# yunqing-me/RICK

Hardware: AMD Instinct MI355X
Metric: G+D train-step images/sec @256px (higher is better)
Workload: dtype f32 (fp16x3 split MFMA, fp32 accumulate); 1 GPU; FFHQ-256 StyleGAN2 G+D RICK iteration (D step, R1/16, G step, PLR/4, EMA, masks on), batch 4/GPU, 256px, channel_multiplier 2, random-init weights; global_batch=4, parallelism=dp1, hip_graphs=True

## Files before the change

include/rick_hip.h:

```cpp
#ifndef RICK_HIP_H
#define RICK_HIP_H

#include <stdint.h>

#ifdef __cplusplus
extern "C" {
#endif

#define RICK_EINVAL 22
#define RICK_MAX_TAPS 16

int rick_abi_version(void);

int rick_upfirdn2d_f32(const float *input, const float *kernel, float *out,
                       int64_t major, int in_h, int in_w, int minor, int kh, int kw,
                       int up_x, int up_y, int down_x, int down_y,
                       int pad_x0, int pad_x1, int pad_y0, int pad_y1, void *stream);

int rick_upfirdn2d_any(const void *input, const void *kernel, void *out, int dtype, int64_t major, int in_h, int in_w,
                       int kh, int kw, int up_x, int up_y, int down_x, int down_y, int pad_x0, int pad_x1, int pad_y0,
                       int pad_y1, void *stream);

int rick_bias_act_f32(const float *x, const float *bias, const float *ref, float *out,
                      int64_t n, int64_t step_b, int64_t size_b, int act, int grad,
// ... 146 lines not shown
int rick_conv_igemm_split_f32(const void *x_split, const float *x_hdr, const void *packed_w, float *out,
                              const float *oscale, const rick_conv_geom *g, const rick_conv_epilogue *epilogue,
                              void *workspace, void *stream);
int rick_convt2_split_f32(const void *x_split, const float *x_hdr, const void *packed_w, float *out, const float *oscale,
                          int N, int IH, int IW, int Ci, int Co, int OH, int OW, float alpha, float *amax ,
                          void *workspace, void *stream);
int rick_conv_wgrad_split_f32(const void *x, const float *x_hdr, const void *gy, const float *gy_hdr, float *gw,
                              int64_t s_co, int64_t s_ci, int64_t s_t, const rick_conv_geom *g, int accumulate,
                              void *workspace, void *stream);

int rick_thin_fwd_f32(const float *x, const float *W, int64_t w_bstride, const float *add,
                      float *t, int N, int64_t P, int C, int J, void *stream);
int rick_thin_bwdx_f32(const float *t, const float *W, int64_t w_bstride, float *x,
                       int N, int64_t P, int C, int J, void *stream);
int rick_torgb_fwd_f32(const float *x, const float *w, const float *s, float wscale, const float *bias,
                       const float *add, float *t, int N, int64_t P, int C, int J, void *stream);
int rick_torgb_bwdx_f32(const float *g, const float *w, const float *s, float wscale, float *gx, int N, int64_t P,
                        int C, int J, void *stream);
int rick_torgb_bwdx_acc_f32(const float *g, const float *w, const float *s, float wscale, float *gx, int N, int64_t P,
                            int C, int J, void *stream);
int rick_thin_wgrad_blocks(int64_t P);
int rick_thin_wgrad_f32(const float *t, const float *x, float *G, int N, int64_t P, int C, int J,
                        float *partials, void *stream);

int rick_chan_scale_f32(const float *x, const float *s, float *y, int N, int64_t P, int C, void *stream);
int rick_hw_dot_blocks(int64_t P);
int rick_hw_dot_f32(const float *a, const float *b, float *d, int N, int64_t P, int C,
                    float *partials, const float *divisor, void *stream);
int rick_hw_dot_scale_f32(const float *a, const float *b, float *d, const float *scale, float *scaled, int N,
                          int64_t P, int C, float *partials, void *stream);
int rick_hw_dot_act_f32(const float *g, const float *y, float *d, int N, int64_t P, int C, const float *bias,
                        const float *noise, const float *noise_w, int noise_nb, float slope, float gain,
                        float *partials, const float *divisor, void *stream);
int rick_add_scale_f32(const float *a, const float *b, float *y, int64_t n, float alpha, void *stream);

int rick_mbstd_fwd_f32(const float *x, float *out, float *stat, int B, int P, int C, int groups, void *stream);
int rick_mbstd_bwd_f32(const float *x, const float *gout, float *gx, int B, int P, int C, int groups, void *stream);

int rick_sq_accumulate_f32(float *acc, const float *g, int64_t n, void *stream);
int rick_filter_reduce_f32(const float *x, float *out, int64_t outer, int64_t outer_stride,
                           int64_t nfilters, int64_t filter_stride, int64_t inner,
                           float scale, void *stream);
int rick_wsq_f32(const float *w, float *wsq, int O, int I, int K, float scale, void *stream);
int rick_demod_f32(const float *s, const float *wsq, float *d, int B, int I, int O, float eps, void *stream);
int rick_demod_bwd_s_f32(const float *s, const float *wsq, const float *d, const float *gd, float *gs, int B, int I, int O,
                         void *stream);
int rick_demod_bwd_w_f32(const float *w, const float *s, const float *d, const float *gd, float *gw, int B, int I, int O,
                         int K, float scale, int accumulate, void *stream);
typedef struct {
    const float *w;
    const float *b;
    int64_t io_off;
    int64_t gw_off, gb_off;
    int C, lat_idx, blk_begin, reserved;
} rick_modbank_desc;
int rick_modbank_blocks(int C);
int rick_modbank_fwd_f32(const float *lat, int B, int n_latent, int K, const rick_modbank_desc *descs_device, int n,
                         int total_blocks, float scale, float *out, void *stream);
int rick_modbank_bwd_f32(const float *lat, const float *gs, int B, int n_latent, int K, const rick_modbank_desc *descs_device,
                         int n, int total_blocks, float scale, float *grad, int accumulate, void *stream);
typedef struct rick_demod_desc {
    const float *w;
    float *wsq;
    float *gw;
    int64_t s_off, d_off;
    int O, I, K;
// ... 134 lines not shown
```

rick_amd/_lib.py:

```python
import ctypes
import os

import torch

_HERE = os.path.dirname(os.path.abspath(__file__))
LIB_PATH = os.path.join(_HERE, 'lib', 'librick_hip.so')
if os.environ.get('RICK_HIP_LIB'):
    import warnings
    LIB_PATH = os.environ['RICK_HIP_LIB']
    warnings.warn(f'rick_amd: RICK_HIP_LIB overrides the product library with {LIB_PATH}', RuntimeWarning)
MAX_TAPS = 16

c_fp = ctypes.c_void_p
c_i64 = ctypes.c_int64
c_int = ctypes.c_int
c_f = ctypes.c_float


class ConvGeom(ctypes.Structure):
    _fields_ = [('N', c_int), ('IH', c_int), ('IW', c_int), ('Ci', c_int),
                ('OH', c_int), ('OW', c_int), ('Co', c_int),
                ('GH', c_int), ('GW', c_int),
                ('is_', c_int), ('os', c_int), ('oy0', c_int), ('ox0', c_int),
                ('ntaps', c_int), ('nslices', c_int),
# ... 71 lines not shown
    'rick_bound_tail_f32': (c_int, [c_fp, c_fp, c_f, c_fp, c_fp, c_fp, c_int, c_f, c_fp, c_int, c_fp]),
    'rick_bias_act_bwd_split2_f32': (c_int, [c_fp, c_fp, c_fp, c_fp, c_fp, c_fp, c_f, c_fp, c_fp, c_fp, c_fp, c_fp, c_fp, c_fp, c_i64,
                                             c_int, c_i64, c_i64, c_i64, c_f, c_f, c_fp, c_int, c_fp]),
    'rick_conv_packed_bytes': (c_i64, [c_int, c_int, c_int]),
    'rick_conv_pack_weight': (c_int, [c_fp, c_i64, c_i64, c_i64, c_int, c_int, c_int, c_f, c_int, c_fp, c_fp]),
    'rick_conv_pack_blocks': (c_int, [c_int, c_int]),
    'rick_conv_pack_weights_multi': (c_int, [c_fp, c_int, c_int, c_int, c_fp]),
    'rick_conv_igemm_workspace_bytes': (c_i64, [ctypes.POINTER(ConvGeom)]),
    'rick_conv_igemm_f32': (c_int, [c_fp, c_fp, c_fp, c_fp, c_fp, ctypes.POINTER(ConvGeom), c_fp, c_fp]),
    'rick_conv_igemm_act_f32': (c_int, [c_fp, c_fp, c_fp, c_fp, c_fp, ctypes.POINTER(ConvGeom),
                                        ctypes.POINTER(ConvEpilogue), c_fp, c_fp]),
    'rick_conv_igemm_multi_workspace_bytes': (c_i64, [ctypes.POINTER(ConvGeom), c_int]),
    'rick_conv_igemm_multi_f32': (c_int, [c_fp, c_fp, c_fp, c_fp, c_fp, ctypes.POINTER(ConvGeom), c_int, c_fp, c_fp]),
    'rick_convt2_workspace_bytes': (c_i64, [c_int] * 7),
    'rick_convt2_plan': (c_int, [c_int] * 7 + [ctypes.POINTER(c_int)]),
    'rick_convt2_posmap': (c_int, [c_int] * 7 + [ctypes.POINTER(ctypes.c_ubyte), ctypes.POINTER(c_int)]),
    'rick_convt2_f32': (c_int, [c_fp, c_fp, c_fp, c_fp, c_fp] + [c_int] * 8 + [c_f, c_fp, c_fp]),
    'rick_conv_wgrad_workspace_bytes': (c_i64, [ctypes.POINTER(ConvGeom)]),
    'rick_conv_wgrad_f32': (c_int, [c_fp, c_fp, c_fp, c_i64, c_i64, c_i64, c_fp, c_fp,
                                    ctypes.POINTER(ConvGeom), c_int, c_fp, c_fp]),
    'rick_thin_fwd_f32': (c_int, [c_fp, c_fp, c_i64, c_fp, c_fp, c_int, c_i64, c_int, c_int, c_fp]),
    'rick_thin_bwdx_f32': (c_int, [c_fp, c_fp, c_i64, c_fp, c_int, c_i64, c_int, c_int, c_fp]),
    'rick_torgb_fwd_f32': (c_int, [c_fp, c_fp, c_fp, c_f, c_fp, c_fp, c_fp, c_int, c_i64, c_int, c_int, c_fp]),
    'rick_torgb_bwdx_f32': (c_int, [c_fp, c_fp, c_fp, c_f, c_fp, c_int, c_i64, c_int, c_int, c_fp]),
    'rick_torgb_bwdx_acc_f32': (c_int, [c_fp, c_fp, c_fp, c_f, c_fp, c_int, c_i64, c_int, c_int, c_fp]),
    'rick_thin_wgrad_blocks': (c_int, [c_i64]),
    'rick_thin_wgrad_f32': (c_int, [c_fp, c_fp, c_fp, c_int, c_i64, c_int, c_int, c_fp, c_fp]),
    'rick_chan_scale_f32': (c_int, [c_fp, c_fp, c_fp, c_int, c_i64, c_int, c_fp]),
    'rick_hw_dot_blocks': (c_int, [c_i64]),
    'rick_hw_dot_f32': (c_int, [c_fp, c_fp, c_fp, c_int, c_i64, c_int, c_fp, c_fp, c_fp]),
    'rick_hw_dot_scale_f32': (c_int, [c_fp, c_fp, c_fp, c_fp, c_fp, c_int, c_i64, c_int, c_fp, c_fp]),
    'rick_hw_dot_act_f32': (c_int, [c_fp, c_fp, c_fp, c_int, c_i64, c_int, c_fp, c_fp, c_fp, c_int, c_f, c_f, c_fp, c_fp,
                                    c_fp]),
    'rick_add_scale_f32': (c_int, [c_fp, c_fp, c_fp, c_i64, c_f, c_fp]),
    'rick_mbstd_fwd_f32': (c_int, [c_fp, c_fp, c_fp, c_int, c_int, c_int, c_int, c_fp]),
    'rick_mbstd_bwd_f32': (c_int, [c_fp, c_fp, c_fp, c_int, c_int, c_int, c_int, c_fp]),
    'rick_sq_accumulate_f32': (c_int, [c_fp, c_fp, c_i64, c_fp]),
    'rick_filter_reduce_f32': (c_int, [c_fp, c_fp, c_i64, c_i64, c_i64, c_i64, c_i64, c_f, c_fp]),
    'rick_masked_adam_f32': (c_int, [c_fp, c_fp, c_fp, c_fp, c_fp, c_i64, c_f, c_f, c_f, c_f, c_f, c_f, c_fp]),
    'rick_wsq_f32': (c_int, [c_fp, c_fp, c_int, c_int, c_int, c_f, c_fp]),
    'rick_demod_f32': (c_int, [c_fp, c_fp, c_fp, c_int, c_int, c_int, c_f, c_fp]),
    'rick_demod_bwd_s_f32': (c_int, [c_fp, c_fp, c_fp, c_fp, c_fp, c_int, c_int, c_int, c_fp]),
    'rick_demod_bwd_w_f32': (c_int, [c_fp, c_fp, c_fp, c_fp, c_fp, c_int, c_int, c_int, c_int, c_f, c_int, c_fp]),
    'rick_colsum_multi_f32': (c_int, [ctypes.POINTER(ColsumItem), c_int, c_fp]),
    'rick_demod_blocks_wsq': (c_int, [c_int, c_int]),
    'rick_demod_blocks': (c_int, [c_int]),
    'rick_demod_blocks_bwd_s': (c_int, [c_int]),
    'rick_wsq_multi_f32': (c_int, [c_fp, c_int, c_int, c_fp]),
    'rick_demod_multi_f32': (c_int, [c_fp, c_fp, c_fp, c_int, c_int, c_int, c_int, c_f, c_fp]),
    'rick_demod_bwd_w_multi_f32': (c_int, [c_fp, c_fp, c_fp, c_fp, c_int, c_int, c_int, c_fp]),
    'rick_demod_bwd_s_multi_f32': (c_int, [c_fp, c_fp, c_fp, c_fp, c_fp, c_int, c_int, c_int, c_int, c_fp]),
    'rick_modbank_blocks': (c_int, [c_int]),
    'rick_modbank_fwd_f32': (c_int, [c_fp, c_int, c_int, c_int, c_fp, c_int, c_int, c_f, c_fp, c_fp]),
    'rick_modbank_bwd_f32': (c_int, [c_fp, c_fp, c_int, c_int, c_int, c_fp, c_int, c_int, c_f, c_fp, c_int, c_fp]),
    'rick_equal_linear_f32': (c_int, [c_fp, c_fp, c_fp, c_fp, c_int, c_int, c_int, c_f, c_f, c_int, c_f, c_f, c_int, c_fp]),
    'rick_linear_fwd_workspace_floats': (c_i64, [c_int, c_int, c_int]),
    'rick_linear_fwd_f32': (c_int, [c_fp, c_fp, c_fp, c_fp, c_int, c_int, c_int, c_f, c_f, c_fp, c_fp]),
    'rick_linear_dgrad_workspace_floats': (c_i64, [c_int, c_int, c_int]),
    'rick_linear_dgrad_f32': (c_int, [c_fp, c_fp, c_fp, c_int, c_int, c_int, c_f, c_fp, c_fp]),
    'rick_linear_wgrad_f32': (c_int, [c_fp, c_fp, c_fp, c_fp, c_int, c_int, c_int, c_f, c_f, c_int, c_fp]),
    'rick_adam_prepare_f32': (c_int, [c_fp, c_int, c_int, c_f, c_f, c_fp, c_fp]),
    'rick_masked_adam_dev_f32': (c_int, [c_fp, c_fp, c_fp, c_fp, c_fp, c_i64, c_f, c_f, c_f, c_f, c_fp, c_fp]),
    'rick_ema_f32': (c_int, [c_fp, c_fp, c_i64, c_f, c_fp]),
    'rick_image_batch_f32': (c_int, [c_fp, c_fp, c_fp, c_fp, c_int, c_int, c_int, c_int, c_fp]),
    'rick_png_unfilter': (c_int, [c_fp, c_int, c_int, c_int]),
    'rick_augment_workspace_floats': (c_i64, [c_int, c_int, c_int]),
# ... 106 lines not shown
```

rick_amd/csrc/elementwise.hip:

```cpp
#include "conv_common.h"

struct BiasActParams {
    int64_t n, step_b, size_b, n_div, hw_div, noise_nb, noise_hw;
    int act, grad;
    float alpha, scale;
};

__device__ __forceinline__ float act_apply(float v, float r, int mode, float alpha) {
    switch (mode) {
        case 30: return v > 0.f ? v : v * alpha;
        case 31: return r > 0.f ? v : v * alpha;
        case 12:
        case 32: return 0.f;
        default: return v;
    }
}

template <bool VEC4>
__global__ __launch_bounds__(256) void bias_act_kernel(const float *__restrict__ x, const float *__restrict__ b,
                                                       const float *__restrict__ ref, float *__restrict__ out,
                                                       const float *__restrict__ noise, const float *__restrict__ nw,
                                                       BiasActParams p) {
    const int mode = p.act * 10 + p.grad;
    const float nwv = noise ? nw[0] : 0.f;
// ... 676 lines not shown
    else
        hipLaunchKernelGGL((hw_dot_kernel<false, false>), dim3(nb, N), dim3(256), 1024 * sizeof(float), st, a, b, partials, P, C, none);
    launch_colsum(partials, d, nb, N * C, N * C, 0, st, divisor);
    RICK_LAUNCH_STATUS();
}

extern "C" int rick_hw_dot_scale_f32(const float *a, const float *b, float *d, const float *scale, float *scaled, int N,
                                     int64_t P, int C, float *partials, void *stream) {
    if (!a || !b || !d || !scale || !scaled || !partials || N <= 0 || P <= 0 || C <= 0 || N > 65535 || (C & 3)) return RICK_EINVAL;
    if (((uintptr_t)a | (uintptr_t)b | (uintptr_t)scale | (uintptr_t)scaled) % 16) return RICK_EINVAL;
    hipStream_t st = (hipStream_t)stream;
    const int nb = rick_hw_dot_blocks(P);
    const HwDotAct t = {nullptr, nullptr, nullptr, 1, 1.f, 1.f, scale, scaled};
    hipLaunchKernelGGL((hw_dot_kernel<true, false, true>), dim3(nb, N), dim3(256), 1024 * sizeof(float), st, a, b, partials, P, C, t);
    launch_colsum(partials, d, nb, N * C, N * C, 0, st);
    RICK_LAUNCH_STATUS();
}

extern "C" int rick_hw_dot_act_f32(const float *g, const float *y, float *d, int N, int64_t P, int C, const float *bias,
                                   const float *noise, const float *noise_w, int noise_nb, float slope, float gain,
                                   float *partials, const float *divisor, void *stream) {
    if (!g || !y || !d || !partials || N <= 0 || P <= 0 || C <= 0 || N > 65535 || (C & 3) || gain == 0.f || slope == 0.f)
        return RICK_EINVAL;
    if ((((uintptr_t)g | (uintptr_t)y | (uintptr_t)(bias ? bias : g)) % 16) || (noise && (!noise_w || (noise_nb != 1 && noise_nb != N))))
        return RICK_EINVAL;
    hipStream_t st = (hipStream_t)stream;
    const int nb = rick_hw_dot_blocks(P);
    const HwDotAct t = {bias, noise, noise_w, noise_nb, 1.f / gain, 1.f / (gain * slope), nullptr, nullptr};
    hipLaunchKernelGGL((hw_dot_kernel<true, true>), dim3(nb, N), dim3(256), 1024 * sizeof(float), st, g, y, partials, P, C, t);
    launch_colsum(partials, d, nb, N * C, N * C, 0, st, divisor);
    RICK_LAUNCH_STATUS();
}

__global__ __launch_bounds__(256) void add_scale_kernel(const float *__restrict__ a, const float *__restrict__ b,
                                                        float *__restrict__ y, int64_t n, float alpha) {
    const int64_t stride = (int64_t)gridDim.x * 256;
    const int64_t n4 = n >> 2;
    for (int64_t i4 = (int64_t)blockIdx.x * 256 + threadIdx.x; i4 < n4; i4 += stride) {
        float4 av = reinterpret_cast<const float4 *>(a)[i4];
        if (b) {
            const float4 bv = reinterpret_cast<const float4 *>(b)[i4];
            av.x += bv.x; av.y += bv.y; av.z += bv.z; av.w += bv.w;
        }
        reinterpret_cast<float4 *>(y)[i4] = make_float4(av.x * alpha, av.y * alpha, av.z * alpha, av.w * alpha);
    }
    for (int64_t i = (n4 << 2) + (int64_t)blockIdx.x * 256 + threadIdx.x; i < n; i += stride)
        y[i] = (a[i] + (b ? b[i] : 0.f)) * alpha;
}

__global__ __launch_bounds__(256) void add_scale_split_kernel(const float *__restrict__ a, const float *__restrict__ b,
                                                              float *__restrict__ y, unsigned char *__restrict__ sy,
                                                              cv_split_hdr *__restrict__ hdr, const float *__restrict__ ba,
                                                              const float *__restrict__ bb, float coef, int64_t n4, float alpha) {
    const cv_split_hdr h = cv_split_header(ba, bb, coef);
    if (blockIdx.x == 0 && threadIdx.x == 0) *hdr = h;
    const float sc = cv_uniform(h.scale);
    float am = 0.f;
    for (int64_t i4 = (int64_t)blockIdx.x * 256 + threadIdx.x; i4 < n4; i4 += (int64_t)gridDim.x * 256) {
        float4 av = reinterpret_cast<const float4 *>(a)[i4];
        const float4 bv = reinterpret_cast<const float4 *>(b)[i4];
        av.x += bv.x; av.y += bv.y; av.z += bv.z; av.w += bv.w;
        const float4 o = make_float4(av.x * alpha, av.y * alpha, av.z * alpha, av.w * alpha);
        reinterpret_cast<float4 *>(y)[i4] = o;
        cv_split_store4(sy + i4 * 16, 0, o, sc);
        am = amax4(am, o);
    }
// ... 219 lines not shown
```

rick_amd/models.py:

```python
import math
import os
import random

import torch
from torch import autograd, nn
from torch.nn import functional as F

from . import op
from .op import modconv as _mc
from .op.fused_act import FusedLeakyReLU, fused_leaky_relu, fused_noise_bias_act
from .op.upfirdn2d import upfirdn2d

CHANNELS = {4: 512, 8: 512, 16: 512, 32: 512}
_USE_DBLOCK = not os.environ.get('RICK_NO_DBLOCK')
_USE_RGB_FORK = not os.environ.get('RICK_NO_RGB_FORK')
_USE_DEMOD_BANK = not os.environ.get('RICK_NO_DEMOD_BANK')
_USE_OWN_LINEAR = not os.environ.get('RICK_NO_OWN_LINEAR')


def _channels(res, channel_multiplier):
    return CHANNELS.get(res, (16384 // res) * channel_multiplier)


def make_kernel(k):
# ... 104 lines not shown
            self.blur = Blur(blur_kernel, pad=((p + 1) // 2 + factor - 1, p // 2 + 1), upsample_factor=factor)
        if downsample:
            factor = 2
            p = (len(blur_kernel) - factor) + (kernel_size - 1)
            self.blur = Blur(blur_kernel, pad=((p + 1) // 2, p // 2))
        self.scale = 1 / math.sqrt(in_channel * kernel_size ** 2)
        self.padding = kernel_size // 2
        self.weight = nn.Parameter(torch.randn(1, out_channel, in_channel, kernel_size, kernel_size))
        self.modulation = EqualLinear(style_dim, in_channel, bias_init=1)
        self.demodulate = demodulate

    def forward(self, x, style, tail=None, s=None, d=None, rgb_tail=None, next_s=None, fork=False):
        if s is None:
            s = self.modulation(style)
        w = self.weight.view(self.out_channel, self.in_channel, self.kernel_size, self.kernel_size)
        if self.kernel_size == 1 and self.out_channel <= 4 and not self.demodulate:
            if rgb_tail is not None and not op.second_order_enabled():
                f = op.torgb_fork if fork else op.torgb
                return f(x, w.view(self.out_channel, self.in_channel), s, rgb_tail[0], rgb_tail[1], self.scale)
            Wn = (self.scale * w.view(1, self.out_channel, self.in_channel)) * s.unsqueeze(1)
            out = op.thin_fwd(x, Wn)
            if rgb_tail is not None:
                out = out + rgb_tail[0]
                out = out + rgb_tail[1] if rgb_tail[1] is not None else out
            return out
        key = (self.weight, 'mod')
        if self.downsample:
            dd = _mc.demod_coeff(w, s, self.scale, self.eps) if self.demodulate else None
            y = op.conv2d(self.blur(op.chan_scale(x, s)), w, 2, 0, wscale=self.scale, key=key)
            return op.chan_scale(y, dd) if dd is not None else y
        if self.demodulate and d is None:
            d = (_mc.demod_coeff(w, s, self.scale, self.eps) if op.second_order_enabled()
                 else _mc.demod_coeff_fused(w, s, self.scale, self.eps, key))
        if op.second_order_enabled():
            y = _mc.modulated_conv_composed(x, w, s, None, self.scale, self.upsample, key)
            if self.upsample:
                y = self.blur(y)
            return op.chan_scale(y, d) if d is not None else y
        if tail is not None and not self.upsample and self.out_channel % 4 == 0:
            return _mc.modulated_conv_fused(x, w, s, d, self.scale, False, key, tail, next_s=next_s)
        y = _mc.modulated_conv_fused(x, w, s, d, self.scale, self.upsample, key)
        if tail is not None and self.upsample:
            return op.upfirdn2d_noise_bias_act(y, self.blur.kernel, self.blur.pad, *tail, next_s=next_s,
                                               bwd_scale=d if _mc._USE_SPLIT else None)
        y = self.blur(y) if self.upsample else y
        return y if tail is None else fused_noise_bias_act(y, *tail)


class NoiseInjection(nn.Module):
    def __init__(self):
        super().__init__()
        self.weight = nn.Parameter(torch.zeros(1))

    def forward(self, image, noise=None):
        if noise is None:
            b, _, h, w = image.shape
            noise = image.new_empty(b, 1, h, w).normal_()
        return image + self.weight * noise


class ConstantInput(nn.Module):
    def __init__(self, channel, size=4):
        super().__init__()
        self.input = nn.Parameter(torch.randn(1, channel, size, size))

    def forward(self, x):
# ... 364 lines not shown
```

rick_amd/op/modconv.py:

```python
import ctypes
import os
import math

import numpy as np
import torch
from torch.autograd import Function

from .._lib import check, lib, ptr, require_cuda_f32, stream_ptr
from .conv import (_conv_launch, _convT_launch, _epilogue, _pack, _sink_target, _wgrad_launch, conv2d, conv_transpose2d,
                   grad_sink_enabled, param_like)
from .misc import _chan_scale_raw, _hw_dot_raw, chan_scale


_USE_SPLIT = bool(__import__('os').environ.get('RICK_GSPLIT'))


_FUSE_ADJOINT_DOT = not os.environ.get('RICK_NO_ADJOINT_DOT')
stats = {'fprop': 0, 'dgrad': 0, 'wgrad': 0, 'produced': 0}


def _bound_tail(w0, c0, gain, nw=None, w_noise=None, bias=None, mul=None):
    from . import split as sp
    out = sp.new_amax(w0.device)
    check(lib.rick_bound_tail_f32(ptr(out), ptr(w0), float(c0), ptr(nw), ptr(w_noise), ptr(bias), bias.numel() if bias is not None else 0,
                                  float(gain), ptr(mul), mul.numel() if mul is not None else 0, stream_ptr()), 'rick_bound_tail_f32')
    return out


def _tensor_amax(t):
    from . import split as sp
    a = sp.taken(t, '_rick_amax')
    return a if a is not None else sp.amax(t)


def _same_tensor(a, b):
    return a is b or (a is not None and b is not None and a.data_ptr() == b.data_ptr() and a.shape == b.shape
                      and a._version == b._version)


def _input_image(x, s):
    from . import split as sp
    img = sp.taken(x, '_rick_split')
    return img if (img is not None and _same_tensor(getattr(img, 'scale_of', None), s)) else None
# ... 276 lines not shown
def _adjoint_with_image(g, y, noise, slope, gain, d, want_b, want_w, sink_b, sink_w):
    from . import split as sp
    from .fused_act import _noise_args
    n, c, h, w = g.shape
    rows = n * h * w
    Ag = _tensor_amax(g)
    bound = _bound_tail(Ag, 1.0, abs(gain) * max(1.0, abs(slope)), mul=d)
    gz = torch.empty_like(g)
    img = sp.SplitImage(torch.empty_like(g), sp.new_words(4, g.device), (bound, None, 1.0))
    img.scale_of = d
    want_w = want_w and noise is not None
    nz, nb, nhw = _noise_args(noise, g) if want_w else (None, 1, 1)
    if (want_b and sink_b is None) or (want_w and sink_w is None):
        sink_b = sink_w = None
    sunk = (want_b and sink_b is not None) or (want_w and sink_w is not None)
    gb = (sink_b if sunk else torch.empty(c, device=g.device, dtype=g.dtype)) if want_b else None
    gw = (sink_w if sunk else torch.empty(1, device=g.device, dtype=g.dtype)) if want_w else None
    part = None
    if want_b or want_w:
        part = torch.empty(lib.rick_bias_act_bwd_blocks(rows, c) * (c + 1), device=g.device, dtype=g.dtype)
    check(lib.rick_bias_act_bwd_split2_f32(ptr(g), ptr(y), ptr(img.data), ptr(img.hdr), None, None, 0.0, None, ptr(d), ptr(bound),
                                           ptr(gz), ptr(gb), ptr(gw), ptr(nz), rows, c, h * w, nb, nhw, float(slope), float(gain),
                                           ptr(part), int(sunk), stream_ptr()), 'rick_bias_act_bwd_split2_f32')
    return gz, img, (None if sunk else gb), (None if sunk else gw)


def modulated_conv_fused(x, w, s, d, wscale, upsample, key=None, tail=None, next_s=None):
    if tail is None:
        return _ModConvFused.apply(x, w, s, d, float(wscale), bool(upsample), key, None, None, None, 0.2, 1.0, None)
    bias, noise, nw, slope, gain = tail
    return _ModConvFused.apply(x, w, s, d, float(wscale), bool(upsample), key, bias, noise, nw, float(slope), float(gain), next_s)


_MB_DESC = np.dtype([('w', '<u8'), ('b', '<u8'), ('io_off', '<i8'), ('gw_off', '<i8'), ('gb_off', '<i8'), ('C', '<i4'),
                     ('lat_idx', '<i4'), ('blk_begin', '<i4'), ('reserved', '<i4')])


class ModulationBank:

    def __init__(self, linears, lat_idx):
        self.linears, self.lat_idx = list(linears), list(lat_idx)
        self.C = [m.weight.shape[0] for m in self.linears]
        self.K = self.linears[0].weight.shape[1]
        self.scale = self.linears[0].scale
        if any(m.weight.shape[1] != self.K or m.scale != self.scale or m.lr_mul != 1 or m.activation for m in self.linears):
            raise RuntimeError('ModulationBank: layers must share style_dim / scale and have no activation')
        self._tables = {}
        self._retired = []
        self.gw_off, self.gb_off, pos = [], [], 0
        for c in self.C:
            self.gw_off.append(pos)
            pos += c * self.K
            self.gb_off.append(pos)
            pos += (c + 3) // 4 * 4
        self.grad_floats = pos
        self.blk_begin, blk = [], 0
        for c in self.C:
            self.blk_begin.append(blk)
            blk += lib.rick_modbank_blocks(c)
        self.total_blocks = blk

    def params(self):
        out = []
        for m in self.linears:
            out += [m.weight, m.bias]
        return out
# ... 306 lines not shown
```

Measured before the change: 173.2 images/s.

## Add fused modulated-conv autograd node for double-backward path-length regularization

Adds a custom autograd node for 3x3 modulated convs when second-order grads are on (the PLR step). It folds the input and output style scaling into the conv launches and provides a hand-written double-backward. That replaces the composed chain of chan_scale, conv and hw_dot ops with fewer kernel launches and fewer intermediate tensors. New fused elementwise kernels (chan_scale2, hw_dot2, hw_dot_axpy) compute combined dot products and scaled sums in one pass. The added complexity risks gradient-correctness bugs, and the path can be disabled with an env var.

Result: no change. 174.3 images/s (median of 6 runs) (+0.6%).

```diff
diff --git a/include/rick_hip.h b/include/rick_hip.h
--- a/include/rick_hip.h
+++ b/include/rick_hip.h
@@ -202,6 +202,12 @@
 int rick_hw_dot_act_f32(const float *g, const float *y, float *d, int N, int64_t P, int C, const float *bias,
                         const float *noise, const float *noise_w, int noise_nb, float slope, float gain,
                         float *partials, const float *divisor, void *stream);
+int rick_chan_scale2_f32(const float *a, const float *sa, const float *b, const float *sb, float *y, int N, int64_t P, int C,
+                         void *stream);
+int rick_hw_dot2_f32(const float *a1, const float *b1, const float *a2, const float *b2, float *d, int N, int64_t P, int C,
+                     float *partials, const float *divisor, void *stream);
+int rick_hw_dot_axpy_f32(const float *a1, const float *b1, const float *a2, float *d, const float *s1, const float *s2,
+                         const float *s2div, float *out, float *out2, int N, int64_t P, int C, float *partials, void *stream);
 int rick_add_scale_f32(const float *a, const float *b, float *y, int64_t n, float alpha, void *stream);
 
 int rick_mbstd_fwd_f32(const float *x, float *out, float *stat, int B, int P, int C, int groups, void *stream);
diff --git a/rick_amd/_lib.py b/rick_amd/_lib.py
--- a/rick_amd/_lib.py
+++ b/rick_amd/_lib.py
@@ -127,6 +127,9 @@
     'rick_hw_dot_scale_f32': (c_int, [c_fp, c_fp, c_fp, c_fp, c_fp, c_int, c_i64, c_int, c_fp, c_fp]),
     'rick_hw_dot_act_f32': (c_int, [c_fp, c_fp, c_fp, c_int, c_i64, c_int, c_fp, c_fp, c_fp, c_int, c_f, c_f, c_fp, c_fp,
                                     c_fp]),
+    'rick_chan_scale2_f32': (c_int, [c_fp, c_fp, c_fp, c_fp, c_fp, c_int, c_i64, c_int, c_fp]),
+    'rick_hw_dot2_f32': (c_int, [c_fp, c_fp, c_fp, c_fp, c_fp, c_int, c_i64, c_int, c_fp, c_fp, c_fp]),
+    'rick_hw_dot_axpy_f32': (c_int, [c_fp, c_fp, c_fp, c_fp, c_fp, c_fp, c_fp, c_fp, c_fp, c_int, c_i64, c_int, c_fp, c_fp]),
     'rick_add_scale_f32': (c_int, [c_fp, c_fp, c_fp, c_i64, c_f, c_fp]),
     'rick_mbstd_fwd_f32': (c_int, [c_fp, c_fp, c_fp, c_int, c_int, c_int, c_int, c_fp]),
     'rick_mbstd_bwd_f32': (c_int, [c_fp, c_fp, c_fp, c_int, c_int, c_int, c_int, c_fp]),
diff --git a/rick_amd/csrc/elementwise.hip b/rick_amd/csrc/elementwise.hip
--- a/rick_amd/csrc/elementwise.hip
+++ b/rick_amd/csrc/elementwise.hip
@@ -732,6 +732,142 @@
     RICK_LAUNCH_STATUS();
 }
 
+__global__ __launch_bounds__(256) void chan_scale2_kernel(const float *__restrict__ a, const float *__restrict__ sa,
+                                                          const float *__restrict__ b, const float *__restrict__ sb,
+                                                          float *__restrict__ y, int64_t PC, int C, int64_t total4) {
+    const int64_t stride = (int64_t)gridDim.x * 256;
+    for (int64_t i4 = (int64_t)blockIdx.x * 256 + threadIdx.x; i4 < total4; i4 += stride) {
+        const int64_t i = i4 << 2;
+        const int64_t n = i / PC;
+        const int c = (int)(i % C);
+        const float4 av = reinterpret_cast<const float4 *>(a)[i4];
+        const float4 bv = reinterpret_cast<const float4 *>(b)[i4];
+        const float4 s = *reinterpret_cast<const float4 *>(sa + n * C + c);
+        const float4 t = *reinterpret_cast<const float4 *>(sb + n * C + c);
+        reinterpret_cast<float4 *>(y)[i4] = make_float4(fmaf(av.x, s.x, bv.x * t.x), fmaf(av.y, s.y, bv.y * t.y),
+                                                        fmaf(av.z, s.z, bv.z * t.z), fmaf(av.w, s.w, bv.w * t.w));
+    }
+}
+
+extern "C" int rick_chan_scale2_f32(const float *a, const float *sa, const float *b, const float *sb, float *y, int N, int64_t P,
+                                    int C, void *stream) {
+    if (!b && !sb) return rick_chan_scale_f32(a, sa, y, N, P, C, stream);
+    if (!a || !sa || !b || !sb || !y || N <= 0 || P <= 0 || C <= 0 || (C & 3)) return RICK_EINVAL;
+    if (((uintptr_t)a | (uintptr_t)sa | (uintptr_t)b | (uintptr_t)sb | (uintptr_t)y) % 16) return RICK_EINVAL;
+    const int64_t total = (int64_t)N * P * C;
+    hipLaunchKernelGGL(chan_scale2_kernel, dim3(ew_grid(total / 4)), dim3(256), 0, (hipStream_t)stream, a, sa, b, sb, y, P * C, C,
+                       total / 4);
+    RICK_LAUNCH_STATUS();
+}
+
+struct HwDot2 {
+    const float *a2, *b2, *s1, *s2, *s2div;
+    float *out, *out2;
+};
+
+template <bool DOT2, bool AXPY>
+__global__ __launch_bounds__(256) void hw_dot2_kernel(const float *__restrict__ a1, const float *__restrict__ b1,
+                                                      float *__restrict__ partials, int64_t P, int C, HwDot2 t) {
+    extern __shared__ float lds[];
+    const int n = blockIdx.y, N = gridDim.y, nb = gridDim.x;
+    const int64_t ppb = cdiv64(P, nb);
+    const int64_t p0 = (int64_t)blockIdx.x * ppb, p1 = p0 + ppb < P ? p0 + ppb : P;
+    const int64_t img = (int64_t)n * P * C;
+    float *pb = partials + ((int64_t)blockIdx.x * N + n) * C;
+    const int ncol = C / 4;
+    for (int cbase = 0; cbase < ncol; cbase += 256) {
+        const int cg = ncol - cbase < 256 ? ncol - cbase : 256;
+        const int rpb = 256 / cg;
+        const int lane_c = threadIdx.x % cg, lane_r = threadIdx.x / cg;
+        float acc[4] = {0.f, 0.f, 0.f, 0.f};
+        if (lane_r < rpb) {
+            const int64_t step = (int64_t)rpb * C;
+            const int col = (cbase + lane_c) * 4;
+            int64_t off = img + (p0 + lane_r) * C + col;
+            float4 u = make_float4(0.f, 0.f, 0.f, 0.f), v = u;
+            if (AXPY) {
+                u = *reinterpret_cast<const float4 *>(t.s1 + (int64_t)n * C + col);
+                v = *reinterpret_cast<const float4 *>(t.s2 + (int64_t)n * C + col);
+                if (t.s2div) {
+                    const float4 q = *reinterpret_cast<const float4 *>(t.s2div + (int64_t)n * C + col);
+                    v = make_float4(v.x / q.x, v.y / q.y, v.z / q.z, v.w / q.w);
+                }
+            }
+            for (int64_t p = p0 + lane_r; p < p1; p += 2 * rpb) {
+                const bool two = p + rpb < p1;
+                float4 av[2], bv[2], cv[2], dv[2];
+#pragma unroll
+                for (int k = 0; k < 2; k++) {
+                    if (k == 0 || two) {
+                        av[k] = *reinterpret_cast<const float4 *>(a1 + off + k * step);
+                        bv[k] = *reinterpret_cast<const float4 *>(b1 + off + k * step);
+                        if (DOT2 || AXPY) cv[k] = *reinterpret_cast<const float4 *>(t.a2 + off + k * step);
+                        if (DOT2) dv[k] = *reinterpret_cast<const float4 *>(t.b2 + off + k * step);
+                    }
+                }
+#pragma unroll
+                for (int k = 0; k < 2; k++) {
+                    if (k == 0 || two) {
+                        acc[0] = fmaf(av[k].x, bv[k].x, acc[0]); acc[1] = fmaf(av[k].y, bv[k].y, acc[1]);
+                        acc[2] = fmaf(av[k].z, bv[k].z, acc[2]); acc[3] = fmaf(av[k].w, bv[k].w, acc[3]);
+                        if (DOT2) {
+                            acc[0] = fmaf(cv[k].x, dv[k].x, acc[0]); acc[1] = fmaf(cv[k].y, dv[k].y, acc[1]);
+                            acc[2] = fmaf(cv[k].z, dv[k].z, acc[2]); acc[3] = fmaf(cv[k].w, dv[k].w, acc[3]);
+                        }
+                        if (AXPY) {
+                            *reinterpret_cast<float4 *>(t.out + off + k * step) =
+                                make_float4(fmaf(bv[k].x, u.x, cv[k].x * v.x), fmaf(bv[k].y, u.y, cv[k].y * v.y),
+                                            fmaf(bv[k].z, u.z, cv[k].z * v.z), fmaf(bv[k].w, u.w, cv[k].w * v.w));
+                            if (t.out2)
+                                *reinterpret_cast<float4 *>(t.out2 + off + k * step) =
+                                    make_float4(av[k].x * v.x, av[k].y * v.y, av[k].z * v.z, av[k].w * v.w);
+                        }
+                    }
+                }
+                off += 2 * step;
+            }
+        }
+        __syncthreads();
+        for (int j = 0; j < 4; j++) lds[threadIdx.x * 4 + j] = lane_r < rpb ? acc[j] : 0.f;
+        __syncthreads();
+        if (threadIdx.x < cg)
+            for (int j = 0; j < 4; j++) {
+                float s = 0.f;
+                for (int rr = 0; rr < rpb; rr++) s += lds[(rr * cg + threadIdx.x) * 4 + j];
+                pb[(cbase + threadIdx.x) * 4 + j] = s;
+            }
+    }
+}
+
+extern "C" int rick_hw_dot2_f32(const float *a1, const float *b1, const float *a2, const float *b2, float *d, int N, int64_t P,
+                                int C, float *partials, const float *divisor, void *stream) {
+    if (!a2 && !b2) return rick_hw_dot_f32(a1, b1, d, N, P, C, partials, divisor, stream);
+    if (!a1 || !b1 || !a2 || !b2 || !d || !partials || N <= 0 || P <= 0 || C <= 0 || N > 65535 || (C & 3)) return RICK_EINVAL;
+    if (((uintptr_t)a1 | (uintptr_t)b1 | (uintptr_t)a2 | (uintptr_t)b2) % 16) return RICK_EINVAL;
+    hipStream_t st = (hipStream_t)stream;
+    const int nb = rick_hw_dot_blocks(P);
+    const HwDot2 t = {a2, b2, nullptr, nullptr, nullptr, nullptr, nullptr};
+    hipLaunchKernelGGL((hw_dot2_kernel<true, false>), dim3(nb, N), dim3(256), 1024 * sizeof(float), st, a1, b1, partials, P, C, t);
+    launch_colsum(partials, d, nb, N * C, N * C, 0, st, divisor);
+    RICK_LAUNCH_STATUS();
+}
+
+extern "C" int rick_hw_dot_axpy_f32(const float *a1, const float *b1, const float *a2, float *d, const float *s1, const float *s2,
+                                    const float *s2div, float *out, float *out2, int N, int64_t P, int C, float *partials,
+                                    void *stream) {
+    if (!a1 || !b1 || !a2 || !d || !s1 || !s2 || !out || !partials || N <= 0 || P <= 0 || C <= 0 || N > 65535 || (C & 3))
+        return RICK_EINVAL;
+    if (((uintptr_t)a1 | (uintptr_t)b1 | (uintptr_t)a2 | (uintptr_t)s1 | (uintptr_t)s2 | (uintptr_t)s2div | (uintptr_t)out |
+         (uintptr_t)out2) % 16)
+        return RICK_EINVAL;
+    hipStream_t st = (hipStream_t)stream;
+    const int nb = rick_hw_dot_blocks(P);
+    const HwDot2 t = {a2, nullptr, s1, s2, s2div, out, out2};
+    hipLaunchKernelGGL((hw_dot2_kernel<false, true>), dim3(nb, N), dim3(256), 1024 * sizeof(float), st, a1, b1, partials, P, C, t);
+    launch_colsum(partials, d, nb, N * C, N * C, 0, st);
+    RICK_LAUNCH_STATUS();
+}
+
 __global__ __launch_bounds__(256) void add_scale_kernel(const float *__restrict__ a, const float *__restrict__ b,
                                                         float *__restrict__ y, int64_t n, float alpha) {
     const int64_t stride = (int64_t)gridDim.x * 256;
diff --git a/rick_amd/models.py b/rick_amd/models.py
--- a/rick_amd/models.py
+++ b/rick_amd/models.py
@@ -160,6 +160,10 @@
         if self.demodulate and d is None:
             d = (_mc.demod_coeff(w, s, self.scale, self.eps) if op.second_order_enabled()
                  else _mc.demod_coeff_fused(w, s, self.scale, self.eps, key))
+        if (op.second_order_enabled() and _mc._PLR_NODE and d is not None and self.kernel_size == 3
+                and (not x.is_cuda or (x.dtype == torch.float32 and self.in_channel % 4 == 0 and self.out_channel % 4 == 0))):
+            y = _mc.modulated_conv_node(x, w, s, d, self.scale, self.upsample, key)
+            return self.blur(y) if self.upsample else y
         if op.second_order_enabled():
             y = _mc.modulated_conv_composed(x, w, s, None, self.scale, self.upsample, key)
             if self.upsample:
diff --git a/rick_amd/op/modconv.py b/rick_amd/op/modconv.py
--- a/rick_amd/op/modconv.py
+++ b/rick_amd/op/modconv.py
@@ -8,7 +8,7 @@
 
 from .._lib import check, lib, ptr, require_cuda_f32, stream_ptr
 from .conv import (_conv_launch, _convT_launch, _epilogue, _pack, _sink_target, _wgrad_launch, conv2d, conv_transpose2d,
-                   grad_sink_enabled, param_like)
+                   grad_sink_enabled, param_like, skip_param_grad)
 from .misc import _chan_scale_raw, _hw_dot_raw, chan_scale
 
 
@@ -351,6 +351,257 @@
     return _ModConvFused.apply(x, w, s, d, float(wscale), bool(upsample), key, bias, noise, nw, float(slope), float(gain), next_s)
 
 
+_PLR_NODE = not os.environ.get('RICK_NO_PLR_NODE')
+
+
+def _bc(t):
+    return t[:, :, None, None]
+
+
+def _al16(t):
+    t = t.contiguous()
+    return t if t.data_ptr() % 16 == 0 else t.clone()
+
+
+def _nhwc16(t):
+    t = t.contiguous(memory_format=torch.channels_last)
+    return t if t.data_ptr() % 16 == 0 else t.clone(memory_format=torch.channels_last)
+
+
+def _host_conv(x, w, wscale, up):
+    import torch.nn.functional as F
+    if up:
+        return F.conv_transpose2d(x, (w * wscale).transpose(0, 1), stride=2)
+    return F.conv2d(x, w * wscale, padding=w.shape[2] // 2)
+
+
+def _node_conv(x, w, wscale, up, key, iscale=None, oscale=None):
+    if not x.is_cuda:
+        y = _host_conv(x * _bc(iscale) if iscale is not None else x, w, wscale, up)
+        return y * _bc(oscale) if oscale is not None else y
+    O, I, kh, kw = w.shape
+    wp = _pack(w, wscale, key and (key[0], key[1] + ('/convT' if up else '/conv')))
+    if up:
+        return _convT_launch(x, wp, O, kh, kw, 2, 0, ((x.shape[2] - 1) * 2 + kh, (x.shape[3] - 1) * 2 + kw), iscale=iscale, oscale=oscale)
+    return _conv_launch(x, wp, O, kh, kw, 1, kh // 2, iscale=iscale, oscale=oscale)
+
+
+def _node_adjoint(g, w, wscale, up, key, hw, iscale):
+    if not g.is_cuda:
+        import torch.nn.functional as F
+        gs = g * _bc(iscale)
+        if up:
+            return F.conv2d(gs, (w * wscale).transpose(0, 1), stride=2)
+        return F.conv_transpose2d(gs, w * wscale, padding=w.shape[2] // 2)
+    O, I, kh, kw = w.shape
+    wpT = _pack(w.transpose(0, 1), wscale, key and (key[0], key[1] + '/T'))
+    if up:
+        return _conv_launch(g, wpT, I, kh, kw, 2, 0, iscale=iscale)
+    return _convT_launch(g, wpT, I, kh, kw, 1, kh // 2, hw, iscale=iscale)
+
+
+def _node_wgrad(terms, w, wscale, up, sink):
+    if not terms:
+        return None
+    O, I, kh, kw = w.shape
+    if not terms[0][0].is_cuda:
+        tot = None
+        for g, gsc, xin, xsc in terms:
+            with torch.enable_grad():
+                wv = torch.zeros_like(w).requires_grad_(True)
+                (gw,) = torch.autograd.grad(_host_conv(xin * _bc(xsc) if xsc is not None else xin, wv, wscale, up), wv, g * _bc(gsc))
+            tot = gw if tot is None else tot + gw
+        if sink is not None:
+            sink.add_(tot)
+            return None
+        return tot
+    acc = sink
+    for g, gsc, xin, xsc in terms:
+        if up:
+            r = _wgrad_launch(xin, g, kh, kw, 2, 0, wscale, ascale=xsc, bscale=gsc, out=acc, transposed=acc is sink and sink is not None)
+        else:
+            r = _wgrad_launch(g, xin, kh, kw, 1, kh // 2, wscale, ascale=gsc, bscale=xsc, out=acc)
+        if acc is None:
+            acc = r
+    if sink is not None:
+        return None
+    return acc.transpose(0, 1) if up else acc
+
+
+def _scale2(a, sa, b=None, sb=None):
+    if not a.is_cuda:
+        return a * _bc(sa) + b * _bc(sb) if b is not None else a * _bc(sa)
+    if b is None:
+        return _chan_scale_raw(a, sa)
+    a, b, sa, sb = _nhwc16(a), _nhwc16(b), _al16(sa), _al16(sb)
+    n, c, h, w = a.shape
+    y = torch.empty_like(a)
+    check(lib.rick_chan_scale2_f32(ptr(a), ptr(sa), ptr(b), ptr(sb), ptr(y), n, h * w, c, stream_ptr()), 'rick_chan_scale2_f32')
+    return y
+
+
+def _dot(a, b, divisor=None):
+    if not a.is_cuda:
+        t = (a * b).sum((2, 3))
+        return t / divisor if divisor is not None else t
+    return _hw_dot_raw(a, b, divisor=divisor)
+
+
+def _dot_axpy(a1, b1, a2, s1, s2, s2div=None, want2=False):
+    if not a1.is_cuda:
+        q = _bc(s2 / s2div if s2div is not None else s2)
+        return (a1 * b1).sum((2, 3)), b1 * _bc(s1) + a2 * q, (a1 * q if want2 else None)
+    a1, b1, a2 = _nhwc16(a1), _nhwc16(b1), _nhwc16(a2)
+    s1, s2 = _al16(s1), _al16(s2)
+    s2div = _al16(s2div) if s2div is not None else None
+    n, c, h, w = a1.shape
+    d = torch.empty((n, c), device=a1.device, dtype=a1.dtype)
+    out = torch.empty_like(b1)
+    out2 = torch.empty_like(a1) if want2 else None
+    part = torch.empty(lib.rick_hw_dot_blocks(h * w) * n * c, device=a1.device, dtype=a1.dtype)
+    check(lib.rick_hw_dot_axpy_f32(ptr(a1), ptr(b1), ptr(a2), ptr(d), ptr(s1), ptr(s2), ptr(s2div), ptr(out), ptr(out2), n, h * w, c,
+                                   ptr(part), stream_ptr()), 'rick_hw_dot_axpy_f32')
+    return d, out, out2
+
+
+def _first_backward(g, x, w, s, d, y, wscale, up, key, need_x, need_s, need_d):
+    gxu = _node_adjoint(g, w, wscale, up, key, (x.shape[2], x.shape[3]), d)
+    gx = gs = gd = None
+    if need_x and need_s and x.is_cuda:
+        gs, gx = _hw_dot_scale_raw(gxu, x, s)
+    else:
+        gs = _dot(gxu, x) if need_s else None
+        gx = _scale2(gxu, s) if need_x else None
+    if need_d:
+        gd = _dot(g, y, divisor=d)
+    return gxu, gx, gs, gd
+
+
+def _first_backward_composed(g, x, w, s, d, y, wscale, up, key):
+    if not x.is_cuda:
+        import torch.nn.functional as F
+        gsc = g * _bc(d)
+        gxu = (F.conv2d(gsc, (w * wscale).transpose(0, 1), stride=2) if up
+               else F.conv_transpose2d(gsc, w * wscale, padding=w.shape[2] // 2))
+        return gxu * _bc(s), (gxu * x).sum((2, 3)), (g * y).sum((2, 3)) / d
+    from .conv import _Conv, _ConvT
+    from .misc import hw_dot
+    kT = key and (key[0], key[1] + '/T')
+    gsc = chan_scale(g, d)
+    if up:
+        gxu = _Conv.apply(gsc, w.transpose(0, 1), 2, 0, wscale, kT)
+    else:
+        gxu = _ConvT.apply(gsc, w.transpose(0, 1), 1, w.shape[2] // 2, wscale, (x.shape[2], x.shape[3]), kT)
+    return chan_scale(gxu, s), hw_dot(gxu, x), hw_dot(g, y) / d
+
+
+def _wgrad_twice(g, x, w, s, d, wscale, up):
+    if not x.is_cuda:
+        with torch.enable_grad():
+            wv = torch.zeros_like(w).requires_grad_(True)
+            (gw,) = torch.autograd.grad(_host_conv(x * _bc(s), wv, wscale, up), wv, g * _bc(d), create_graph=True)
+        return gw
+    from .conv import _WGrad
+    kh, kw = w.shape[2], w.shape[3]
+    if up:
+        return _WGrad.apply(chan_scale(x, s), chan_scale(g, d), kh, kw, 2, 0, wscale).transpose(0, 1)
+    return _WGrad.apply(chan_scale(g, d), chan_scale(x, s), kh, kw, 1, kh // 2, wscale)
+
+
+class _ModConvNode(Function):
+
+    @staticmethod
+    def forward(ctx, x, w, s, d, wscale, upsample, key):
+        y = _node_conv(x, w, wscale, upsample, key, iscale=_al16(s), oscale=_al16(d))
+        ctx.save_for_backward(x, w, s, d, y)
+        ctx.cfg = (wscale, upsample, key, grad_sink_enabled(), param_like(w))
+        return y
+
+    @staticmethod
+    def backward(ctx, g):
+        x, w, s, d, y = ctx.saved_tensors
+        wscale, up, key, sink, w_param = ctx.cfg
+        need_x, need_w, need_s, need_d = ctx.needs_input_grad[:4]
+        need_w = need_w and not skip_param_grad(w_param)
+        gw = None
+        if torch.is_grad_enabled():
+            gx, gs, gd = _ModConvBwd.apply(g, x, w, s, d, y, wscale, up, key, sink, need_x, need_s, need_d)
+            if need_w:
+                gw = _wgrad_twice(g, x, w, s, d, wscale, up)
+        else:
+            sc, dc = _al16(s), _al16(d)
+            _, gx, gs, gd = _first_backward(g, x, w, sc, dc, y, wscale, up, key, need_x, need_s, need_d)
+            if need_w:
+                gw = _node_wgrad([(g, dc, x, sc)], w, wscale, up, _sink_target(key, w.shape, sink))
+        return gx, gw, gs, gd, None, None, None
+
+
+class _ModConvBwd(Function):
+
+    @staticmethod
+    def forward(ctx, g, x, w, s, d, y, wscale, upsample, key, sink, need_x, need_s, need_d):
+        s, d = _al16(s), _al16(d)
+        gxu, gx, gs, gd = _first_backward(g, x, w, s, d, y, wscale, upsample, key, need_x, need_s, need_d)
+        ctx.save_for_backward(g, x, w, s, d, y, gxu, gd)
+        ctx.cfg = (wscale, upsample, key, sink, param_like(w))
+        ctx.set_materialize_grads(False)
+        return gx, gs, gd
+
+    @staticmethod
+    def backward(ctx, cx, cs, cd):
+        g, x, w, s, d, y, gxu, gd = ctx.saved_tensors
+        wscale, up, key, sink, w_param = ctx.cfg
+        need_g, need_x, need_w, need_s, need_d, need_y = ctx.needs_input_grad[:6]
+        need_w = need_w and not skip_param_grad(w_param)
+        tail = (None,) * 7
+        if torch.is_grad_enabled():
+            from ._twice import second_order_backward
+            res = second_order_backward(
+                lambda g_, x_, w_, s_, d_, y_: _first_backward_composed(g_, x_, w_, s_, d_, y_, wscale, up, key),
+                (g, x, w, s, d, y), (need_g, need_x, need_w, need_s, need_d, need_y), (cx, cs, cd),
+                (False, False, w_param, False, False, False))
+            return (*res, *tail)
+        cs = _al16(cs) if cs is not None else None
+        cd = _al16(cd) if cd is not None else None
+        v = z = None
+        if cx is not None or cs is not None:
+            v = _scale2(cx, s, x, cs) if (cx is not None and cs is not None) else _scale2(cx, s) if cx is not None else _scale2(x, cs)
+            if need_g or need_d:
+                z = _node_conv(v, w, wscale, up, key)
+        cot_g = cot_x = cot_s = cot_d = cot_y = None
+        if z is not None and cd is not None:
+            cot_d, cot_g, cot_y = _dot_axpy(g, z, y, d, cd, d, want2=need_y)
+        elif z is not None:
+            if x.is_cuda:
+                cot_d, cot_g = _hw_dot_scale_raw(z, g, d)
+            else:
+                cot_d, cot_g = _dot(z, g), _scale2(z, d)
+        elif cd is not None:
+            q = cd / d
+            cot_g = _scale2(y, q) if need_g else None
+            cot_y = _scale2(g, q) if need_y else None
+        if cd is not None and need_d:
+            cot_d = -(cd * gd / d) if cot_d is None else cot_d - cd * gd / d
+        if cx is not None and cs is not None and x.is_cuda:
+            cot_s, cot_x = _hw_dot_scale_raw(gxu, cx, cs)
+        else:
+            cot_s = _dot(cx, gxu) if (cx is not None and need_s) else None
+            cot_x = _scale2(gxu, cs) if (cs is not None and need_x) else None
+        cot_w = None
+        if need_w and v is not None:
+            cot_w = _node_wgrad([(g, d, v, None)], w, wscale, up, _sink_target(key, w.shape, sink))
+        return (cot_g if need_g else None, cot_x if need_x else None, cot_w, cot_s if need_s else None,
+                cot_d if need_d else None, cot_y if need_y else None, *tail)
+
+
+def modulated_conv_node(x, w, s, d, wscale, upsample, key=None):
+    if x.is_cuda:
+        require_cuda_f32(x, w, s, d)
+        if w.shape[0] % 4 or w.shape[1] % 4:
+            raise RuntimeError('modulated_conv_node: channel counts must be multiples of 4')
+    return _ModConvNode.apply(x, w, s, d, float(wscale), bool(upsample), key)
+
+
 _MB_DESC = np.dtype([('w', '<u8'), ('b', '<u8'), ('io_off', '<i8'), ('gw_off', '<i8'), ('gb_off', '<i8'), ('C', '<i4'),
                      ('lat_idx', '<i4'), ('blk_begin', '<i4'), ('reserved', '<i4')])
 
```
